# anibali/dsnt-pose2d

Hardware: AMD Instinct MI355X
Metric: images/sec (train step, 256x256, 16 joints) (higher is better)
Workload: dtype f32; 1 GPU; hg2 + DSNT + JS reg, 256x256 -> 64x64x16, batch 32 per GPU, RMSprop lr 2.5e-4, train step fwd+loss+bwd+optim; global_batch=32, parallelism=dp1, launches_fwd=212

## Files before the change

### dsnt-pose2d_amd/csrc/api.cpp

```cpp
#include "common.h"
#include "stage.h"
#include <string.h>

static thread_local char g_err[512] = "";

int dsnt_set_error(int code, const char* fmt, ...) {
    va_list ap;
    va_start(ap, fmt);
    vsnprintf(g_err, sizeof(g_err), fmt, ap);
    va_end(ap);
    return code;
}

int dsnt_device_id(void) {
    int d = 0;
    if (hipGetDevice(&d) != hipSuccess || d < 0) d = 0;
    return d < DSNT_MAX_DEVICES ? d : DSNT_MAX_DEVICES - 1;
}

int dsnt_device_cus(void) {
    static std::atomic<int> cus[DSNT_MAX_DEVICES];
    const int d = dsnt_device_id();
    int c = cus[d].load(std::memory_order_acquire);
    if (!c) {
        hipDeviceProp_t prop;
        int dev = 0;
        c = (hipGetDevice(&dev) == hipSuccess && hipGetDeviceProperties(&prop, dev) == hipSuccess && prop.multiProcessorCount > 0)
                ? prop.multiProcessorCount : 256;
        cus[d].store(c, std::memory_order_release);
    }
    return c;
}

extern "C" int dsnt_version(void) { return 124; }
extern "C" const char* dsnt_last_error(void) { return g_err; }

#include <vector>
#include <new>

struct dsnt_list {
    struct Entry {
        int kind;
        int lane, src, dst;
        mutable hipEvent_t ev;
        std::function<void(hipStream_t)> fn;
        int st_code = 0, gx = 0, gy = 0, nt = 0;
        std::vector<unsigned char> params;
        int fused = 0;
        unsigned* st_sync = nullptr;
    };
    std::vector<Entry> entries;
    std::vector<size_t> seg_start;
    dsnt_list() { seg_start.push_back(0); }
};

static thread_local dsnt_list* g_rec = nullptr;

dsnt_list* dsnt_recording(void) { return g_rec; }

void dsnt_record_launch(dsnt_list* l, int lane, std::function<void(hipStream_t)>&& fn) {
    dsnt_list::Entry e;
    e.kind = 0; e.lane = lane; e.src = e.dst = 0; e.ev = nullptr; e.fn = std::move(fn);
    l->entries.push_back(std::move(e));
}

void dsnt_record_launch_op(dsnt_list* l, int lane, std::function<void(hipStream_t)>&& fn, int code, int gx, int gy, int nt,
                           const void* params, size_t bytes) {
    dsnt_list::Entry e;
    e.kind = 0; e.lane = lane; e.src = e.dst = 0; e.ev = nullptr; e.fn = std::move(fn);
    if (code > 0 && code < DSNT_ST_CODES && bytes <= DSNT_STAGE_PARAM_BYTES && gx > 0 && gy > 0 && (nt == 256 || nt == DSNT_STAGE_NT || nt == 1024)) {
        e.st_code = code; e.gx = gx; e.gy = gy; e.nt = nt;
        e.params.assign((const unsigned char*)params, (const unsigned char*)params + bytes);
    }
    l->entries.push_back(std::move(e));
}

struct StageRun { std::vector<size_t> idx; int lane; int max_vb; };

static void stage_runs(const dsnt_list* l, int min_run, int max_vgrid, std::vector<StageRun>& runs) {
    std::vector<StageRun> open(DSNT_MAX_LANES);
    for (int i = 0; i < DSNT_MAX_LANES; ++i) { open[i].lane = i; open[i].max_vb = 0; }
    auto close = [&](int lane) {
        if ((int)open[lane].idx.size() >= min_run) runs.push_back(open[lane]);
        open[lane].idx.clear(); open[lane].max_vb = 0;
    };
    size_t next_seg = 1;
    for (size_t i = 0; i < l->entries.size(); ++i) {
// ... 164 lines not shown
```

### dsnt-pose2d_amd/csrc/conv_epilogue.h

```cpp
#pragma once
#include "conv_split.h"

template <int WM, int WN, int TM, int TN, bool HALO = false, int NT = 512>
__device__ __forceinline__ void conv_epilogue(const ConvP& p, f32x16 (&acc)[TM][TN], float* smem, int mtile,
                                              int ntile, int tid, int wave, int lane, int mbase = 0) {
    constexpr int BM = WM * TM * 32, BN = WN * TN * 32;
    auto rowmap = [&](int row) {
        return HALO ? mbase + (row >> 4) * p.W + (((row & 15) + ((row >> 4) & 1) * 14) & 15) : mtile * BM + row;
    };
    const int lr = lane & 31, lh = lane >> 5;
    const int cw = wave & 3;
    const int wm = cw / WN, wn = cw % WN;
    constexpr int CP = BN + 4;
    float* Cs = smem;
    if (wave < 4) {
#pragma unroll
        for (int a = 0; a < TM; ++a)
#pragma unroll
            for (int b = 0; b < TN; ++b) {
                const int col = (wn * TN + b) * 32 + lr;
                const int row0 = (wm * TM + a) * 32 + 4 * lh;
#pragma unroll
                for (int e = 0; e < 16; ++e)
                    Cs[(row0 + (e & 3) + 8 * (e >> 2)) * CP + col] = acc[a][b][e];
// ... 2 lines not shown
    __syncthreads();
    constexpr int CH = BN / 4;
    constexpr int RPP = NT / CH;
    constexpr int NPT = BM / RPP;
    constexpr int NP = NPT > 8 ? 8 : NPT;
    constexpr int NG = NPT / NP;
    const int ch = tid % CH, r0 = tid / CH;
    const int n0 = ntile * BN + ch * 4;
    const bool vn = n0 < p.Cout;
    float4 bias4 = make_float4(0.f, 0.f, 0.f, 0.f);
    if (p.bias && vn) bias4 = *reinterpret_cast<const float4*>(p.bias + n0);
    const bool bnb = p.bnb_scale != nullptr;
    float4 bsc = bias4, bsh = bias4, bmu = bias4, bis = bias4;
    if (bnb && vn) {
        bsc = *reinterpret_cast<const float4*>(p.bnb_scale + n0);
        bsh = *reinterpret_cast<const float4*>(p.bnb_shift + n0);
        bmu = *reinterpret_cast<const float4*>(p.bnb_mean + n0);
        bis = *reinterpret_cast<const float4*>(p.bnb_invstd + n0);
    } else if (p.tail.amax_bn && vn) {
        bsc = *reinterpret_cast<const float4*>(p.tail.amax_scale + n0);
        bsh = *reinterpret_cast<const float4*>(p.tail.amax_shift + n0);
    }
    const float am2lo = p.tail.amax_relu ? 0.f : -__builtin_inff();
    float am2 = 0.f;
    const float osc = p.a_bound ? 1.f / (pow2_scale(bound64(p.a_bound)) * pow2_scale(bound64(p.w_bound))) : 1.f;
    float4 s1 = make_float4(0.f, 0.f, 0.f, 0.f), s2 = s1;
    float am = 0.f;
#pragma unroll
    for (int gi = 0; gi < NG; ++gi) {
    float4 r1[NP], r2[NP];
#pragma unroll
    for (int j = 0; j < NP; ++j) {
        const int m = rowmap(r0 + RPP * (gi * NP + j));
        const bool ok = vn && m < p.M;
        const size_t o = ok ? (size_t)m * p.Cout + n0 : 0;
        r1[j] = p.res1 ? *reinterpret_cast<const float4*>(p.res1 + o) : make_float4(0.f, 0.f, 0.f, 0.f);
        r2[j] = p.res2 ? *reinterpret_cast<const float4*>(p.res2 + o) : make_float4(0.f, 0.f, 0.f, 0.f);
    }
#pragma unroll
    for (int j = 0; j < NP; ++j) {
        const int row = r0 + RPP * (gi * NP + j);
        const int m = rowmap(row);
        if (vn && m < p.M) {
            float4 v = *reinterpret_cast<const float4*>(Cs + row * CP + ch * 4);
            v.x *= osc; v.y *= osc; v.z *= osc; v.w *= osc;
            if (bnb) {
                const float4 xv = r1[j];
                if (p.bnb_relu) {
                    if (fmaf(xv.x, bsc.x, bsh.x) <= 0.f) v.x = 0.f;
                    if (fmaf(xv.y, bsc.y, bsh.y) <= 0.f) v.y = 0.f;
                    if (fmaf(xv.z, bsc.z, bsh.z) <= 0.f) v.z = 0.f;
                    if (fmaf(xv.w, bsc.w, bsh.w) <= 0.f) v.w = 0.f;
                }
                *reinterpret_cast<float4*>(p.y + (size_t)m * p.Cout + n0) = v;
                s1.x += v.x; s1.y += v.y; s1.z += v.z; s1.w += v.w;
                s2.x = fmaf(v.x, (xv.x - bmu.x) * bis.x, s2.x); s2.y = fmaf(v.y, (xv.y - bmu.y) * bis.y, s2.y);
                s2.z = fmaf(v.z, (xv.z - bmu.z) * bis.z, s2.z); s2.w = fmaf(v.w, (xv.w - bmu.w) * bis.w, s2.w);
                am = fmaxf(fmaxf(am, fabsf(v.x)), fmaxf(fabsf(v.y), fmaxf(fabsf(v.z), fabsf(v.w))));
                continue;
            }
            v.x += bias4.x + r1[j].x + r2[j].x; v.y += bias4.y + r1[j].y + r2[j].y;
            v.z += bias4.z + r1[j].z + r2[j].z; v.w += bias4.w + r1[j].w + r2[j].w;
            *reinterpret_cast<float4*>(p.y + (size_t)m * p.Cout + n0) = v;
            am = fmaxf(fmaxf(am, fabsf(v.x)), fmaxf(fabsf(v.y), fmaxf(fabsf(v.z), fabsf(v.w))));
            if (p.tail.amax_bn)
                am2 = fmaxf(fmaxf(am2, fabsf(fmaxf(fmaf(v.x, bsc.x, bsh.x), am2lo))),
                            fmaxf(fabsf(fmaxf(fmaf(v.y, bsc.y, bsh.y), am2lo)),
                                  fmaxf(fabsf(fmaxf(fmaf(v.z, bsc.z, bsh.z), am2lo)), fabsf(fmaxf(fmaf(v.w, bsc.w, bsh.w), am2lo)))));
            s1.x += v.x; s1.y += v.y; s1.z += v.z; s1.w += v.w;
            s2.x = fmaf(v.x, v.x, s2.x); s2.y = fmaf(v.y, v.y, s2.y);
            s2.z = fmaf(v.z, v.z, s2.z); s2.w = fmaf(v.w, v.w, s2.w);
        }
    }
    }
    if (p.tail.amax) amax_commit(am, p.tail.amax);
    if (p.tail.amax_bn) amax_commit(am2, p.tail.amax_bn, 1);
    if (p.stats) {
        __syncthreads();
        float* red = smem;
        float* mine = red + ((size_t)r0 * BN + ch * 4) * 2;
        mine[0] = s1.x; mine[1] = s2.x; mine[2] = s1.y; mine[3] = s2.y;
        mine[4] = s1.z; mine[5] = s2.z; mine[6] = s1.w; mine[7] = s2.w;
        __syncthreads();
        if (tid < BN) {
            const int n = ntile * BN + tid;
            if (n < p.Cout) {
                float a0 = 0.f, a1 = 0.f;
#pragma unroll
                for (int w = 0; w < RPP; ++w) {
                    a0 += red[((size_t)w * BN + tid) * 2 + 0];
                    a1 += red[((size_t)w * BN + tid) * 2 + 1];
                }
                tail_store(p.stats + ((size_t)mtile * 2 + 0) * p.Cout + n, a0);
                tail_store(p.stats + ((size_t)mtile * 2 + 1) * p.Cout + n, a1);
            }
        }
    }
}
```

### dsnt-pose2d_amd/csrc/conv_f32.hip

```cpp
#include "conv_epilogue.h"
#include "ew_bodies.h"
#include "stage.h"
#include <string.h>
#include <stdlib.h>

#define BK 32
#define PITCH 36

template <int WM, int WN, int TM, int TN, bool PRO, bool FAST>
__global__ __launch_bounds__(512, 4) void conv_fwd_kernel(ConvP p) {
    constexpr int BM = WM * TM * 32, BN = WN * TN * 32;
    constexpr int APASS = BM / 32, BPASS = BN / 32;
    extern __shared__ __attribute__((aligned(16))) float smem[];
    float* As = smem;
    float* Bs = smem + 2 * BM * PITCH;

    int tile;
    xcd_remap(blockIdx.x, p.mtiles * p.ntiles, tile);
    const int ntile = tile % p.ntiles, mtile = tile / p.ntiles;

    const int tid = threadIdx.x, lane = tid & 63;
    const int wave = __builtin_amdgcn_readfirstlane(tid >> 6);
    const int nsteps = (p.K + BK - 1) / BK;
    const int lr = lane & 31, lh = lane >> 5;
// ... 443 lines not shown
                p.y[o] = v;
                s1 += v;
                s2 = fmaf(v, (xv - bmu) * bis, s2);
            } else {
                v += bias + (PRO ? (p.res1 ? p.res1[o] : 0.f) : r1v[j]) + (p.res2 ? p.res2[o] : 0.f);
                p.y[o] = v;
                s1 += v;
                s2 = fmaf(v, v, s2);
            }
        }
    }
    if (p.stats) {
        __syncthreads();
        float* red = &part[0][0][0];
        red[(rg * 32 + col) * 2 + 0] = s1;
        red[(rg * 32 + col) * 2 + 1] = s2;
        __syncthreads();
        if (tid < 32 && vn) {
            float a0 = 0.f, a1 = 0.f;
#pragma unroll
            for (int w = 0; w < 16; ++w) { a0 += red[(w * 32 + tid) * 2 + 0]; a1 += red[(w * 32 + tid) * 2 + 1]; }
            tail_store(p.stats + ((size_t)mtile * 2 + 0) * p.Cout + n, a0);
            tail_store(p.stats + ((size_t)mtile * 2 + 1) * p.Cout + n, a1);
        }
    }
}
template <bool PRO, int CW>
__global__ __launch_bounds__(512) void conv_ksplit_kernel(ConvP p) {
    __shared__ __attribute__((aligned(16))) float part[8][32][33];
    conv_ksplit_body<PRO, CW>(p, blockIdx.x, part, true);
}

static long ksplit_rows() {
    static long v = -1;
    if (v < 0) {
        const char* e = getenv("DSNT_X_KSPLIT_ROWS");
        v = e ? atol(e) : 2048;
    }
    return v;
}

static bool conv_fwd_pro_ok(const dsnt_conv_geom* g, int tiles, int C) {
    return g && C == g->Cin && C <= 256 && C % 4 == 0 && tiles > 0 && (long)tiles * C <= 16384;
}
extern "C" int dsnt_conv_fwd_pro_ok(const dsnt_conv_geom* g, int tiles, int C) { return conv_fwd_pro_ok(g, tiles, C) ? 1 : 0; }

int conv_fill(ConvP& p, const char* who, const float* x, const void* w, bool planes, int64_t plane_stride, const float* bias,
              float* y, const float* in_scale, const float* in_shift, int in_relu, const float* res1, const float* res2,
              float* stats_partial, const dsnt_conv_geom* g, const dsnt_bn_bwd_epilogue* bnb, const dsnt_out_bounds* tail) {
    if (int e = conv_check_geom(g, who)) return e;
    char who_ex[64];
    snprintf(who_ex, sizeof(who_ex), "%s_ex", who);
    DSNT_REQUIRE(!bnb || (bnb->x && bnb->scale && bnb->shift && bnb->mean && bnb->invstd &&
                          stats_partial && !res1 && !res2 && !bias), DSNT_ERR_ARG,
                 "%s: the batch-norm-backward epilogue needs x/scale/shift/mean/invstd and "
                 "stats_partial, and excludes bias/residuals", who_ex);
    DSNT_REQUIRE(x && w && y, DSNT_ERR_ARG, "%s: null tensor", who);
    DSNT_REQUIRE((in_scale == nullptr) == (in_shift == nullptr), DSNT_ERR_ARG,
                 "%s: in_scale/in_shift must be given together", who);
    DSNT_REQUIRE(!planes || dsnt_conv_bf16x6_ok(g), DSNT_ERR_SHAPE,
                 "%s: geometry not supported (need Cin %% 16 == 0, <= 16 taps, < 2 GiB)", who);
    DSNT_REQUIRE(dsnt_aligned16(x) && dsnt_aligned16(w) && (!in_scale || dsnt_aligned16(in_scale)) &&
                 (!in_shift || dsnt_aligned16(in_shift)), DSNT_ERR_ALIGN,
                 "%s: x/w/scale/shift must be 16-byte aligned", who);
    DSNT_REQUIRE(!planes || (plane_stride >= (int64_t)g->Cout * g->R * g->S * g->Cin && plane_stride % 8 == 0 &&
                             (2 * plane_stride + (int64_t)g->Cout * g->R * g->S * g->Cin) * 2 < (1LL << 31)), DSNT_ERR_SHAPE,
                 "%s: bad plane stride %lld", who, (long long)plane_stride);
    p.x = x; p.bias = bias; p.y = y; p.in_scale = in_scale; p.in_shift = in_shift;
    p.w = planes ? nullptr : (const float*)w;
    p.wq = planes ? (const unsigned short*)w : nullptr; p.wq_stride = planes ? plane_stride : 0;
    p.res1 = res1; p.res2 = res2; p.stats = stats_partial; p.in_relu = in_relu;
    p.bnb_scale = p.bnb_shift = p.bnb_mean = p.bnb_invstd = nullptr; p.bnb_relu = 0;
    p.a_bound = p.w_bound = nullptr;
    p.ap_y = p.ap_scale = p.ap_mean = p.ap_invstd = p.ap_coef = nullptr; p.ap_out = nullptr;
    if (bnb) {
        p.res1 = bnb->x; p.bnb_scale = bnb->scale; p.bnb_shift = bnb->shift;
        p.bnb_mean = bnb->mean; p.bnb_invstd = bnb->invstd; p.bnb_relu = bnb->relu;
    }
    if (int e = out_bounds_fill(p.tail, tail, who_ex)) return e;
    DSNT_REQUIRE(!(p.tail.amax_bn && bnb), DSNT_ERR_ARG, "%s: dsnt_out_bounds.amax_bn excludes the batch-norm-backward epilogue", who_ex);
    memset(&p.pro, 0, sizeof(p.pro));
    conv_geom_fill(p, g);
    return DSNT_OK;
}

static int conv_fwd_impl(const float* x, const float* w, const float* bias, float* y,
                         const float* in_scale, const float* in_shift, int in_relu,
                         const float* res1, const float* res2, float* stats_partial,
                         const dsnt_conv_geom* g, const dsnt_bn_bwd_epilogue* g_bnb, const dsnt_out_bounds* g_tail,
                         void* stream, const dsnt_bn_prologue* g_pro = nullptr) {
    ConvP p;
    if (int e = conv_fill(p, "dsnt_conv_fwd", x, w, false, 0, bias, y, in_scale, in_shift, in_relu, res1, res2, stats_partial, g,
                          g_bnb, g_tail)) return e;
    if (g_pro) {
        DSNT_REQUIRE(g_pro->partial && g_pro->mean && g_pro->invstd && g_pro->scale && g_pro->shift && g_pro->M > 0 &&
                     conv_fwd_pro_ok(g, g_pro->tiles, g_pro->C), DSNT_ERR_ARG,
                     "dsnt_conv_fwd_pro: incomplete dsnt_bn_prologue, or more than 256 channels / 128 KB of partial sums");
        DSNT_REQUIRE((g_pro->running_mean == nullptr) == (g_pro->running_var == nullptr), DSNT_ERR_ARG,
                     "dsnt_conv_fwd_pro: running_mean/var must be given together");
        DSNT_REQUIRE(dsnt_aligned16(g_pro->scale) && dsnt_aligned16(g_pro->shift), DSNT_ERR_ALIGN, "dsnt_conv_fwd_pro: alignment");
        p.pro.partial = g_pro->partial; p.pro.tiles = g_pro->tiles; p.pro.C = g_pro->C;
        p.pro.invM = 1.0 / (double)g_pro->M;
        p.pro.unbias = g_pro->M > 1 ? (double)g_pro->M / (double)(g_pro->M - 1) : 1.0;
        p.pro.gamma = g_pro->gamma; p.pro.beta = g_pro->beta; p.pro.rmean = g_pro->running_mean; p.pro.rvar = g_pro->running_var;
        p.pro.momentum = g_pro->momentum; p.pro.eps = g_pro->eps;
        p.pro.mean = g_pro->mean; p.pro.invstd = g_pro->invstd; p.pro.scale = g_pro->scale; p.pro.shift = g_pro->shift;
    }
    int BM, BN;
    pick_cfg(g, BM, BN);
// ... 124 lines not shown
```

### dsnt-pose2d_amd/dsnt/engine.py

```python
import ctypes as C
import os
import struct

import torch

from . import _lib
from ._lib import ConvGeom, BnBwdEpilogue, BnTail, BnPrologue, BnBwdApply

BN_EPS = 1e-5
BN_MOMENTUM = 0.1


class Act:
    __slots__ = ('buf', 'N', 'H', 'W', 'C', '_grad', 'stats', 'name', 'grad_amax', 'amax_tail', 'fold_ok',
                 'pending_apply', 'uses', 'gives_away', 'is_branch', 'grad_shared', 'pending_add', 'base', 'base_amax')

    def __init__(self, buf, name=''):
        self.buf = buf
        self.N, self.H, self.W, self.C = buf.shape
        self._grad = None
        self.base, self.base_amax = None, None
        self.stats = None
        self.amax_tail = None
        self.grad_amax = None
        self.fold_ok = False
        self.pending_apply = None
        self.uses = 0
        self.gives_away = False
        self.is_branch = False
        self.grad_shared = False
        self.pending_add = None
        self.name = name

    @property
    def M(self):
        return self.N * self.H * self.W

    @property
    def grad(self):
        if self._grad is None and self.base is not None:
            self._grad, self.grad_amax, self.grad_shared = self.base, self.base_amax, True
        return self._grad

    @grad.setter
    def grad(self, g):
        self._grad = g


class ConvParams:
    __slots__ = ('w', 'b', 'gw', 'gb', 'Cout', 'R', 'S', 'Cin', 'stride', 'pad', 'dil', 'wq', 'wq_stride', 'wq16', 'wb',
                 'post_reduce')

    def __init__(self, w, b, gw, gb, stride=1, pad=0, dil=1):
        self.w, self.b, self.gw, self.gb = w, b, gw, gb
        self.wq, self.wq_stride = None, 0
        self.wq16, self.wb = None, None
        self.post_reduce = None
        self.Cout, self.R, self.S, self.Cin = w.shape
        self.stride, self.pad, self.dil = stride, pad, dil


class BnParams:
    __slots__ = ('gamma', 'beta', 'ggamma', 'gbeta', 'rmean', 'rvar', 'C', 'uses', 'momentum', 'eps')

    def __init__(self, gamma, beta, ggamma, gbeta, rmean, rvar, momentum=BN_MOMENTUM, eps=BN_EPS):
        self.gamma, self.beta, self.ggamma, self.gbeta = gamma, beta, ggamma, gbeta
        self.rmean, self.rvar = rmean, rvar
        self.momentum, self.eps = float(momentum), float(eps)
        self.C = gamma.numel()
        self.uses = 0


class Normed:
    __slots__ = ('x', 'bn', 'mean', 'invstd', 'scale', 'shift', 'relu', 'abound', 'pending', 'lane')


class _Conv:
    __slots__ = ('src', 'x', 'y', 'p', 'g', 'res1', 'res2', 'name', 'normed', 'sc', 'sh', 'relu', 'x_amax', 'use6', 'use16',
                 'slot', 'slot_k', 'bucket', 'fuse1', 'fold3_ok', 'need_input_grad', 'gd')


class _Dgrad:
    __slots__ = ('native', 'gd', 'gsrc', 'wd', 'wq', 'wq_stride', 'wq16', 'wbd', 'g_amax', 'd6', 'd16', 'd_stream')


class Tape:
    def __init__(self, device, training, record=None):
        self.device = device
        self.training = training
        self.record = training if record is None else bool(record)
        self.fwd = []
        self.bwd = []
        self._bwd_emitters = []
        self._scratch = {}
        self._keep = []
        self.lib = _lib.load()
        self.nbytes = 0
        self.bytes_fwd, self.bytes_bwd, self.bytes_by_name, self._ws_ptrs = 0, 0, {}, set()
        self._read_switches()
        self.lane = 0
        self.side_stream, self.wgrad_stream, self.more_streams = None, None, ()
        self.stage_census = []
        self._f16_w_stream = {}
        self.cur_bucket = 0
        self._wgrad_lane_reads = set()
        self._writer_base = None
        self._ident = None
        self._release_total, self._release_left, self._held = 0, 0, []
        self.acts = []
        self.dgrad_slots = []
        self.dgrad_total, self.dgrad_f32, self.dgrad_planes = 0, None, None
        self.param_arena = None
        self._pending_reduce = []
        self._pending_group = []
        self._f16_w_rows, self._f16_w_seen = [], set()
        self._f16_bn_rows = []
        self._eval_bn_rows = []
        self._amax_buf, self._amax_used = None, 0
        self._planar_src, self._prep_exempt, self._post_reduce = {}, set(), []
        self._famax_buf, self._famax_used, self._famax_of, self._famax_bn_of = None, 0, {}, {}
        self._f16_dw_rows = []
        self._dgrad_pack = None
        self.dgrad_planes16, self.dgrad_bounds = None, None
        self.f16_uses = []
        self._pending_group_uses = []
        self._clists = {}

    def _read_switches(self):
        self.use_bf16x6 = os.environ.get('DSNT_MFMA', 'bf16x6') != 'f32'
        self.bf16x6_min_rows = int(os.environ.get('DSNT_BF16X6_MIN_ROWS', '4096'))
        self.use_lanes = os.environ.get('DSNT_LANES', '1') != '0'
        self.side_lanes = (1, 3)
        self.n_lanes = 3 + len(self.side_lanes) - 1
        self.chain_lanes = (0,) + self.side_lanes
        self.wgrad_lane = 2 if (self.use_lanes and os.environ.get('DSNT_WGRAD_LANE', '1') != '0') else None
        self.wgrad_lane_rows = int(os.environ.get('DSNT_X_WGRAD_LANE_ROWS', '16000'))
        self.release_rows = int(os.environ.get('DSNT_X_RELEASE_ROWS', '4096'))
        off = set(os.environ.get('DSNT_OFF', '').replace('+', ',').split(','))
        self.conv3s = 'conv3s' not in off
        self.bwd1 = 'bwd1' not in off
        self.fwd1 = 'fwd1' not in off
        self.fold3 = 'fold3' not in off
        self.fold3_rows = int(os.environ.get('DSNT_X_FOLD3_ROWS', '16384'))
        self.stem4 = 'stem4' not in off
        self.stage = os.environ.get('DSNT_STAGE', '0') == '1'
        self.stage_min_run = int(os.environ.get('DSNT_X_STAGE_MIN_RUN', '3'))
        self.stage_max_vgrid = int(os.environ.get('DSNT_X_STAGE_MAX_VGRID', '512'))
        self.stage_grid = int(os.environ.get('DSNT_X_STAGE_GRID', '64'))
        self._x = dict(kv.split('=') for kv in os.environ.get('DSNT_X', '').split(',') if '=' in kv)
        self.wgrad_narrow = self._x.get('wgrad_narrow', '1')
        self.share_grads = self._x.get('share_grads', '1') != '0'
        self.defer_res = self._x.get('defer_res', '1') != '0'
        self.flush_points = self._x.get('flush_points', '1') != '0'
        self.prep_split = self._x.get('prep_split', '1') != '0'
        self.defer_reduce = os.environ.get('DSNT_DEFER_REDUCE', '1') != '0'
        self.group_rows = int(os.environ.get('DSNT_X_GROUP_ROWS', '8192')) if self.defer_reduce else 0
        self.fuse_finalize = os.environ.get('DSNT_FUSE_FINALIZE', '1') != '0'
        self.fuse_finalize_max = int(os.environ.get('DSNT_X_FUSE_FINALIZE_MAX', '2048'))
        self.use_f16x3 = self.use_bf16x6 and os.environ.get('DSNT_SPLIT', 'f16x3') == 'f16x3'
        if self.record and not self.training:
            self.use_f16x3 = False

    def empty(self, *shape, dtype=torch.float32):
        t = torch.empty(*shape, device=self.device, dtype=dtype)
        self.nbytes += t.numel() * t.element_size()
        self._keep.append(t)
        return t

    def scratch(self, key, numel, dtype=torch.float32, least=1):
        key = (key, self.lane)
        t = self._scratch.get(key)
        if t is None or t.numel() < numel:
            if t is not None:
                self._keep.append(t)
            t = torch.empty(max(numel, least), device=self.device, dtype=dtype)
            self.nbytes += t.numel() * t.element_size()
            self._scratch[key] = t
        return t

    def f16_weights(self, p, wq16=None, wsrc=None, wb=None, stream=False):
        wq16 = p.wq16 if wq16 is None else wq16
        key = wq16.data_ptr()
        if key not in self._f16_w_seen:
            self._f16_w_seen.add(key)
            wsrc = p.w if wsrc is None else wsrc
            wb = p.wb if wb is None else wb
            n = wsrc.numel()
            assert n % 4 == 0
            self._f16_w_rows.append([wsrc.data_ptr(), wq16.data_ptr(), wb.data_ptr(), n, p.wq_stride] +
                                    ([p.Cout, p.Cin] if stream else [0, 0]))
            self._f16_w_stream[key] = stream
        assert self._f16_w_stream.get(key, False) == stream, 'one weight tensor, two plane layouts'

    def stream_ok(self, p, g, rows, res2):
        return (self.conv3s and p.R == 3 and p.S == 3 and res2 is None and
                bool(self.lib.dsnt_conv_fwd_stream_ok(C.byref(g))))
# ... 409 lines not shown
        acc = 1
        if a.grad is None:
            a.grad = self.empty(a.N, a.H, a.W, a.C)
            acc = 0
        elif a.grad.data_ptr() in self._wgrad_lane_reads:
            self._wgrad_lane_reads.discard(a.grad.data_ptr())
            self.release_wgrads()
            self.sync_bwd(self.wgrad_lane, self.lane)
        if self.use_f16x3 and amax:
            if a.grad_amax is None:
                a.grad_amax = self.amax_slot()
        else:
            a.grad_amax = None
        return a.grad, acc

    def grad_identity(self, a, g, donate, g_amax=None):
        if a.pending_apply is not None:
            self.materialize_apply(a)
        if a.pending_add is not None:
            self._flush_add(a)
        if a.grad is None and donate:
            a.grad = g
            a.grad_amax = g_amax
            return True
        buf, acc = self.grad_target(a, amax=True)
        if a.grad_amax is not None:
            self.b('dsnt_axpy_amax', g, buf, 1.0, acc, g.numel(), a.grad_amax)
        else:
            self.b('dsnt_axpy', g, buf, 1.0, acc, g.numel())
        return False

    def geom(self, x, p):
        Ho = (x.H + 2 * p.pad - p.dil * (p.R - 1) - 1) // p.stride + 1
        Wo = (x.W + 2 * p.pad - p.dil * (p.S - 1) - 1) // p.stride + 1
        assert x.C == p.Cin, (x.C, p.Cin)
        return ConvGeom(x.N, x.H, x.W, p.Cin, Ho, Wo, p.Cout, p.R, p.S, p.stride, p.pad, p.dil)

    def ensure_stats(self, a):
        if a.stats is None:
            tiles = (a.M + 127) // 128
            part = self.empty(tiles, 2, a.C)
            self.f('dsnt_bn_stats', a.buf, part, a.M, a.C)
            a.stats = (part, tiles)
        return a.stats

    def norm(self, x, bn, relu=True):
        if os.environ.get('DSNT_DEBUG_NO_RELU'):
            relu = False
        n = Normed()
        n.x, n.bn, n.relu = x, bn, relu
        n.abound = None
        n.mean, n.invstd, n.scale, n.shift = (self.empty(bn.C) for _ in range(4))
        n.pending = None
        n.lane = self.lane
        if self.training:
            part, tiles = self.ensure_stats(x)
            if self.fuse_finalize and bn.C <= 256 and tiles * bn.C <= self.fuse_finalize_max:
                n.pending = (part, tiles)
            else:
                self.f('dsnt_bn_finalize', part, tiles, x.M, bn.C, bn.gamma, bn.beta, bn.rmean, bn.rvar,
                       bn.momentum, bn.eps, 1, n.mean, n.invstd, n.scale, n.shift)
        else:
            bits = struct.unpack('<I', struct.pack('<f', float(bn.eps)))[0]
            self._eval_bn_rows.append([bn.gamma.data_ptr(), bn.beta.data_ptr(), bn.rmean.data_ptr(), bn.rvar.data_ptr(),
                                       n.mean.data_ptr(), n.invstd.data_ptr(), n.scale.data_ptr(), n.shift.data_ptr(),
                                       bn.C, bits])
        return n

    def check_lane(self, n):
        if n.pending is not None:
            n.lane = self.lane
        elif n.lane != self.lane:
            raise RuntimeError('dsnt: BatchNorm vectors finalised on lane %d are read on lane %d without a synchronisation '
                               '(trace norm() and its consumers on one lane, or sync the lanes)' % (n.lane, self.lane))

    def materialize(self, n):
        self.check_lane(n)
        if n.pending is not None:
            part, tiles = n.pending
            n.pending = None
            bn = n.bn
            self.f('dsnt_bn_finalize', part, tiles, n.x.M, bn.C, bn.gamma, bn.beta, bn.rmean, bn.rvar,
                   bn.momentum, bn.eps, 1, n.mean, n.invstd, n.scale, n.shift)

    def fold_ok(self, n):
        x = n.x
        return bool(self.bwd1 and x.fold_ok and x.grad is None and x.pending_apply is None)

    def materialize_apply(self, x):
        ap, x.pending_apply = x.pending_apply, None
        n = ap['n']
        buf, acc = self.grad_target(x, amax=True)
        if x.grad_amax is not None:
            self.b('dsnt_bn_act_bwd_apply_amax', ap['dz'], x.buf, n.scale, n.shift, n.mean, n.invstd, ap['coef'], 0,
                   buf, acc, x.M, n.bn.C, x.grad_amax)
        else:
            self.b('dsnt_bn_act_bwd_apply', ap['dz'], x.buf, n.scale, n.shift, n.mean, n.invstd, ap['coef'], 0,
                   buf, acc, x.M, n.bn.C)

    def _norm_backward(self, n, da, reduced=None, finalised=False, dz_amax=None):
        x, bn = n.x, n.bn
        coef = self.scratch('bncoef', 2 * bn.C)
        relu = 1 if n.relu else 0
        if reduced is not None:
            part, tiles = reduced
            relu = 0
        else:
            tiles = (x.M + 127) // 128
            part = self.scratch('bnpart', tiles * 2 * bn.C).view(-1)
            self.b('dsnt_bn_act_bwd_reduce', da, x.buf, n.scale, n.shift, n.mean, n.invstd, relu, part,
                   x.M, bn.C)
        if dz_amax is not None:
            assert reduced is not None and not finalised and x.grad is None
            acc_p = 1 if bn.uses > 0 else 0
            bn.uses += 1
            coef = self.empty(2 * bn.C)
            bound = self.amax_slot()
            self.b('dsnt_bn_bwd_finalize_bound', part, tiles, x.M, bn.C, bn.ggamma, bn.gbeta, acc_p, coef, n.scale,
                   dz_amax, bound)
            x.pending_apply = dict(dz=da, n=n, coef=coef, bound=bound, dz_amax=dz_amax)
            return
        frozen = not self.training
        fused = (not finalised) and self.fuse_finalize and bn.C <= 256 and tiles * bn.C <= self.fuse_finalize_max and not frozen
        assert not (frozen and finalised)
        if not finalised:
            acc_p = 1 if bn.uses > 0 else 0
            bn.uses += 1
            if not fused:
                self.b('dsnt_bn_bwd_finalize', part, tiles, x.M, bn.C, bn.ggamma, bn.gbeta, acc_p | (2 if frozen else 0), coef)
        buf, acc = self.grad_target(x, amax=True, base_ok=True)
        base = self.take_base()
        if fused:
            coef = self.empty(2 * bn.C)
            if base is not None:
                self.b('dsnt_bn_act_bwd_apply_pro_base', da, x.buf, n.scale, n.shift, n.mean, n.invstd, part, tiles,
                       bn.ggamma, bn.gbeta, acc_p, coef, relu, base, buf, x.M, bn.C, x.grad_amax)
            else:
                self.b('dsnt_bn_act_bwd_apply_pro', da, x.buf, n.scale, n.shift, n.mean, n.invstd, part, tiles,
                       bn.ggamma, bn.gbeta, acc_p, coef, relu, buf, acc, x.M, bn.C, x.grad_amax)
        elif base is not None:
            self.b('dsnt_bn_act_bwd_apply_base', da, x.buf, n.scale, n.shift, n.mean, n.invstd, coef, relu,
                   base, buf, x.M, bn.C, x.grad_amax)
        elif x.grad_amax is not None:
            self.b('dsnt_bn_act_bwd_apply_amax', da, x.buf, n.scale, n.shift, n.mean, n.invstd, coef, relu,
                   buf, acc, x.M, bn.C, x.grad_amax)
        else:
            self.b('dsnt_bn_act_bwd_apply', da, x.buf, n.scale, n.shift, n.mean, n.invstd, coef, relu,
                   buf, acc, x.M, bn.C)

    def conv(self, src, p, res1=None, res2=None, want_stats=False, need_input_grad=True, name=''):
        c = _Conv()
        c.src, c.p, c.res1, c.res2, c.name, c.need_input_grad = src, p, res1, res2, name, need_input_grad
        c.normed = isinstance(src, Normed)
        c.x = x = src.x if c.normed else src
        c.g = self.geom(x, p)
        c.y = y = self.act(x.N, c.g.Ho, c.g.Wo, p.Cout, name)
        x.uses += 1
        for r in (res1, res2):
            if r is not None:
                r.uses += 1
                y.gives_away = True
        c.sc, c.sh, c.relu = (src.scale, src.shift, 1 if src.relu else 0) if c.normed else (None, None, 0)
        self._conv_forward(c, want_stats)
        if self.record:
            self._conv_backward_plan(c)
            self.on_backward(lambda: self._conv_backward(c))
        return y

    def _share(self, persistent=True):
        return 2 if (persistent and self.lane != 0) else 0

    def _operand_bound(self, c):
        return self.operand_amax_bn(c.src) if c.normed else self.operand_amax(c.x)

    @staticmethod
    def _bn_epilogue(x, n):
        vectors = (n.scale, n.shift, n.mean, n.invstd) if n is not None else (None,) * 4
        return BnBwdEpilogue(_lib.ptr(x.buf), *(_lib.ptr(v) for v in vectors), 1 if (n is not None and n.relu) else 0)

    @staticmethod
    def _bn_apply(y, ap):
        n = ap['n']
        return (BnBwdApply(_lib.ptr(y.buf), _lib.ptr(n.scale), _lib.ptr(n.mean), _lib.ptr(n.invstd), _lib.ptr(ap['coef'])),
                dict(dz=ap['dz'], y=y.buf, scale=n.scale, mean=n.mean, invstd=n.invstd, coef=ap['coef']))

    def _dz_buffer(self, x, private):
        n = x.M * x.C
        return self.empty(n) if private else self.scratch('da', n).view(-1)[:n]

    def _reduce_row(self, ws, p, splits):
        self._pending_reduce.append([ws.data_ptr(), p.gw.data_ptr(), p.gb.data_ptr() if p.gb is not None else 0,
                                     splits, p.Cout * p.R * p.S * p.Cin, p.Cout, 0])

    def _struct_bytes(self, name, nb):
        self.bytes_bwd += nb
        self.bytes_by_name[name] = self.bytes_by_name.get(name, 0) + nb

    def _conv_forward(self, c, want_stats):
        src, x, y, p, g, normed, res2 = c.src, c.x, c.y, c.p, c.g, c.normed, c.res2
        sc, sh, relu = c.sc, c.sh, c.relu
        if normed:
            self.check_lane(src)
        part, tail = None, None
        use6 = c.use6 = self._use6(g) and p.wq is not None
        can16 = use6 and p.wq16 is not None
        early = can16 and p.R == 1 and res2 is None and self.fwd1
        x_amax = self._operand_bound(c) if early else None
# ... 26 lines not shown
            ab = self.f16_bn_bound(src) if (normed and self.training) else x_amax
            if f1:
                e = self.f('dsnt_conv1x1_fwd_f16x3', x.buf, p.wq16, p.wq_stride, p.wb, ab, p.b, y.buf, sc, sh, relu | f1_shr, r1,
                           part, g, tail)
            elif s4:
                e = self.f('dsnt_stem4_fwd_f16x3', x.buf, p.wq16, p.wq_stride, p.wb, ab, p.b, y.buf, part, g, tail)
            else:
                e = self.f('dsnt_conv_fwd_f16x3_stream' if st else 'dsnt_conv_fwd_f16x3_ex', x.buf, p.wq16, p.wq_stride, p.wb, ab,
                           p.b, y.buf, sc, sh, relu | self._share(st or p.R == 1), r1, r2, part, g, None, tail)
            self.f16_uses.append((e, dict(kind='fwd', name=c.name, x=x.buf, sc=sc, sh=sh, relu=relu, a_bound=ab,
                                          w=p.w, w_bound=p.wb)))
        elif use6:
            self.f('dsnt_conv_fwd_bf16x6_ex', x.buf, p.wq, p.wq_stride, p.b, y.buf, sc, sh, relu, r1, r2, part, g,
                   None, tail)
        elif normed and src.pending is not None and self.lib.dsnt_conv_fwd_pro_ok(C.byref(g), src.pending[1], src.bn.C):
            spart, stiles = src.pending
            src.pending = None
            bn = src.bn
            pro = BnPrologue(_lib.ptr(spart), stiles, bn.C, x.M, _lib.ptr(bn.gamma), _lib.ptr(bn.beta), _lib.ptr(bn.rmean),
                             _lib.ptr(bn.rvar), bn.momentum, bn.eps, _lib.ptr(src.mean), _lib.ptr(src.invstd),
                             _lib.ptr(src.scale), _lib.ptr(src.shift))
            self._keep.extend((spart, src.mean, src.invstd, src.scale, src.shift))
            self.f('dsnt_conv_fwd_pro', x.buf, p.w, p.b, y.buf, pro, relu, r1, r2, part, g, tail)
        else:
            if normed:
                self.materialize(src)
            self.f('dsnt_conv_fwd_ex', x.buf, p.w, p.b, y.buf, sc, sh, relu, r1, r2, part, g, None, tail)

    def _conv_backward_plan(self, c):
        x, y, p, g = c.x, c.y, c.p, c.g
        c.slot = c.slot_k = None
        if c.need_input_grad and self.param_arena is not None:
            c.slot, c.slot_k = self.dgrad_total, len(self.dgrad_slots)
            self.dgrad_slots.append((p, c.slot))
            self.dgrad_total += (p.w.numel() + 7) // 8 * 8
        c.bucket = self.cur_bucket
        one_pass = self.bwd1 and self.use_f16x3 and self.defer_reduce and c.slot is not None
        c.fuse1 = bool(one_pass and (c.normed or c.x_amax is not None) and p.R == 1 and p.S == 1 and p.post_reduce is None and
                       self.lib.dsnt_conv1x1_bwd_ok(C.byref(g)))
        plain = c.normed and c.res1 is None and c.res2 is None
        c.gd = None
        if p.stride == 1:
            c.gd = ConvGeom(x.N, g.Ho, g.Wo, p.Cout, x.H, x.W, p.Cin, p.R, p.S, 1, p.dil * (p.R - 1) - p.pad, p.dil)
        c.fold3_ok = bool(self.fold3 and one_pass and plain and self.training and p.R == 3 and p.S == 3 and c.gd is not None and
                          c.use16 and y.M >= self.fold3_rows and self._use6(c.gd) and self.stream_ok(p, c.gd, x.M, None))
        y.fold_ok = bool(c.fuse1 and plain) or c.fold3_ok

    def _conv_backward(self, c):
        y = c.y
        gy, ap = y.grad, y.pending_apply
        fused = c.fuse1 and self.dgrad_planes16 is not None
        fold3 = bool(c.fold3_ok and ap is not None and gy is None and self.dgrad_planes16 is not None and c.need_input_grad and
                     ap['bound'] is not None)
        if ap is not None and (not fused or gy is not None) and not fold3:
            self.materialize_apply(y)
            ap, gy = None, y.grad
        assert gy is not None or ap is not None, 'no gradient reached conv output ' + c.name
        if fused and ap is None and y.grad_amax is None:
            fused = False
        wl, defer_res = self.lane, False
        if fused:
            self._conv_bwd_fused1(c, ap, gy)
        elif fold3:
            gy = y._grad = self.empty(y.N, y.H, y.W, y.C)
            y.grad_amax, y.pending_apply = ap['bound'], None
            self._conv_dgrad(c, gy, ap)
            wl, defer_res = self._conv_wgrad(c, gy)
        else:
            wl, defer_res = self._conv_wgrad(c, gy)
            self._conv_dgrad(c, gy, None)
        self._conv_residual_grads(c, gy, wl, defer_res)

    def _conv_bwd_fused1(self, c, ap, gy):
        src, x, y, p, g, name = c.src, c.x, c.y, c.p, c.g, 'dsnt_conv1x1_bwd_f16x3'
        nw = p.w.numel()
        shr = self._share()
        nsp = self.lib.dsnt_conv1x1_bwd_splits(C.byref(g), shr)
        ws = self.empty(self.lib.dsnt_conv1x1_bwd_ws_floats(C.byref(g), shr))
        self._ws_ptrs.add(ws.data_ptr())
        wd = self.dgrad_f32[c.slot:c.slot + nw]
        wq16 = self.dgrad_planes16[c.slot:c.slot + nw]
        wbd = self.dgrad_bounds[64 * c.slot_k:64 * c.slot_k + 64]
        self._f16_dw_rows.append([wd.data_ptr(), wq16.data_ptr(), wbd.data_ptr(), nw, self.dgrad_total, 0, 0])
        if ap is not None:
            aps, applied = self._bn_apply(y, ap)
            dy, gb = ap['dz'], ap['bound']
            y.pending_apply = None
            grad = dict(g_apply=applied, g_bound=gb)
        else:
            aps, dy, gb = None, gy, y.grad_amax
            grad = dict(g=dy, g_bound=gb)
        if c.normed:
            ab = self.f16_bn_bound_bwd(src)
            fold = self.fold_ok(src)
            dz = self._dz_buffer(x, fold)
            dz_amax = self.amax_slot() if fold else None
            part = self.scratch('bnpart', nsp * 2 * x.C).view(-1)
            e = self.b(name, self._bn_epilogue(x, src), dy, aps, wq16, self.dgrad_total, wbd, ab, gb, dz, part, ws, dz_amax, shr, g)
        else:
            ab = c.x_amax
            buf, acc = self.grad_target(x, amax=True)
            e = self.b(name, self._bn_epilogue(x, None), dy, None, wq16, self.dgrad_total, wbd, ab, gb, buf, None, ws,
                       x.grad_amax, shr | acc, g)
        self._struct_bytes(name, 4 * (x.buf.numel() + (y.buf.numel() if ap is not None else 0)))
        u = dict(kind='bwd1', name=c.name, x=x.buf, sc=c.sc, sh=c.sh, relu=c.relu, a_bound=ab, w=wd, w_bound=wbd)
        u.update(grad)
        self.f16_uses.append((e, u))
        self._reduce_row(ws, p, nsp)
        if c.normed:
            self._norm_backward(src, dz, reduced=(part, nsp), finalised=False, dz_amax=dz_amax)

    def _conv_wgrad(self, c, gy):
        p, g = c.p, c.g
        cur = wl = self.lane
        if self.wgrad_lane is not None and (self.wgrad_lane_rows == 0 or (
                cur in self.chain_lanes and c.res1 is None and c.res2 is None and g.N * g.Ho * g.Wo >= self.wgrad_lane_rows)):
            wl = self.wgrad_lane
        hold = wl != cur and self._release_left > 0
        if hold:
            listed, self.bwd = self.bwd, self._held
        self.sync_bwd(cur, wl)
        self.lane = wl
        if wl != cur:
            self._wgrad_lane_reads.add(gy.data_ptr())
        share = 2 if (wl != cur and c.need_input_grad) else 0
        if share and self.wgrad_narrow in ('1', {0: '2'}.get(c.bucket, '3')):
            share |= 4
        w6 = self.use_bf16x6 and bool(self.lib.dsnt_conv_wgrad_bf16x6_ok(C.byref(g)))
        defer_res = False
        if self.defer_reduce:
            defer_res = self._conv_wgrad_slab(c, gy, share, w6, wl == cur)
        else:
            ws = self.scratch('wgrad', self.lib.dsnt_conv_wgrad_ws_floats(C.byref(g)))
            self.b('dsnt_conv_wgrad_bf16x6' if w6 else 'dsnt_conv_wgrad', c.x.buf, c.sc, c.sh, c.relu, gy, ws, p.gw, p.gb, 0, g)
            if p.post_reduce is not None:
                self.b(p.post_reduce[0], *p.post_reduce[1])
        self.lane = cur
        if hold:
            self.bwd = listed
        return wl, defer_res

    def _conv_wgrad_slab(self, c, gy, share, w6, on_chain):
        x, y, p, g, normed, sc, sh, relu = c.x, c.y, c.p, c.g, c.normed, c.sc, c.sh, c.relu
        groupable = (w6 and (normed or self.share_grads) and on_chain and not y.grad_shared and
                     0 < g.N * g.Ho * g.Wo <= self.group_rows)
        residuals = [r for r in (c.res1, c.res2) if r is not None]
        defer_res = bool(groupable and residuals and self.share_grads and self.defer_res and all(
            r._grad is None and r.base is None and r.pending_apply is None and r.pending_add is None for r in residuals))
        grouped = groupable and (not residuals or defer_res)
        w16 = w6 and self.use_f16x3 and (normed or c.x_amax is not None) and y.grad_amax is not None
        ab = (self.f16_bn_bound_bwd(c.src) if normed else c.x_amax) if w16 else None
        if w16 and not grouped:
            nws = self.lib.dsnt_conv_wgrad_f16x3_ws_floats(C.byref(g), share)
            splits = self.lib.dsnt_conv_wgrad_f16x3_splits(C.byref(g), share)
        else:
            nws, splits = self.lib.dsnt_conv_wgrad_ws_floats(C.byref(g)), self.lib.dsnt_conv_wgrad_splits(C.byref(g))
        ws = self.empty(nws)
        self._ws_ptrs.add(ws.data_ptr())
        use = dict(kind='wgrad', name=c.name, x=x.buf, sc=sc, sh=sh, relu=relu, a_bound=ab, g=gy, g_bound=y.grad_amax)
        if grouped:
            desc = C.create_string_buffer(self.lib.dsnt_conv_wgrad_desc_bytes())
            gsc, gsh = (sc, sh) if normed else self.identity_bn(x.C)
            if w16:
# ... 2 lines not shown
                self._pending_group_uses.append(use)
            else:
                nblk = self.lib.dsnt_conv_wgrad_desc(_lib.ptr(x.buf), _lib.ptr(gsc), _lib.ptr(gsh), relu, _lib.ptr(gy),
                                                     _lib.ptr(ws), C.byref(g), desc)
            if nblk <= 0:
                raise RuntimeError('dsnt_conv_wgrad_desc failed: %s' % self.lib.dsnt_last_error().decode())
            self._pending_group.append((desc.raw, nblk))
        elif w16:
            e = self.b('dsnt_conv_wgrad_f16x3', x.buf, sc, sh, relu, gy, ws, None, None, share, ab, y.grad_amax, g)
            self.f16_uses.append((e, use))
        else:
            self.b('dsnt_conv_wgrad_bf16x6' if w6 else 'dsnt_conv_wgrad', x.buf, sc, sh, relu, gy, ws, None, None,
                   share if w6 else 0, g)
        if p.post_reduce is not None:
            self._post_reduce.append(p.post_reduce)
        self._reduce_row(ws, p, splits)
        return defer_res

    def _conv_dgrad_operands(self, c, gy):
        x, p, g = c.x, c.p, c.g
        d = _Dgrad()
        nw = p.w.numel()
        pad_d = p.dil * (p.R - 1) - p.pad
        assert pad_d >= 0, 'data gradient needs pad <= dil * (R - 1)'
        d.native = p.stride != 1 and c.slot is not None and self.lib.dsnt_conv_dgrad_strided_ok(C.byref(g))
        d.gd, d.gsrc = c.gd, gy
        if p.stride != 1 and not d.native:
            Hs, Ws = x.H + 2 * p.pad - p.dil * (p.R - 1), x.W + 2 * p.pad - p.dil * (p.S - 1)
            d.gsrc = self.scratch('stuffed', x.N * Hs * Ws * p.Cout).view(-1)[:x.N * Hs * Ws * p.Cout]
            self.b('dsnt_zero_insert', gy, d.gsrc, x.N, g.Ho, g.Wo, p.Cout, Hs, Ws, p.stride)
            d.gd = ConvGeom(x.N, Hs, Ws, p.Cout, x.H, x.W, p.Cin, p.R, p.S, 1, pad_d, p.dil)
        d.wq = d.wq_stride = d.wq16 = d.wbd = d.d_stream = None
        if c.slot is not None:
            d.wd = self.dgrad_f32[c.slot:c.slot + nw]
            d.wq, d.wq_stride = self.dgrad_planes[c.slot:c.slot + nw], self.dgrad_total
            d.d6 = d.gd is not None and self._use6(d.gd)
        else:
            d.wd = self.scratch('wdgrad', nw)
            self.b('dsnt_conv_pack_dgrad', p.w, d.wd, p.Cout, p.R, p.S, p.Cin)
            d.d6 = self._use6(d.gd) and nw % 8 == 0
            if d.d6:
                d.wq, d.wq_stride = self.scratch('wdgrad6', 3 * nw, torch.bfloat16, 8), nw
                self.b('dsnt_split_bf16x3', d.wd, d.wq, nw)
        d.g_amax = c.y.grad_amax if (self.use_f16x3 and p.stride == 1) else None
        d.d16 = d.d6 and d.g_amax is not None and c.slot is not None and self.dgrad_planes16 is not None
        if d.d16:
            d.wq16 = self.dgrad_planes16[c.slot:c.slot + nw]
            d.wbd = self.dgrad_bounds[64 * c.slot_k:64 * c.slot_k + 64]
            d.d_stream = self.stream_ok(p, d.gd, x.M, None)
            self._f16_dw_rows.append([d.wd.data_ptr(), d.wq16.data_ptr(), d.wbd.data_ptr(), nw, self.dgrad_total] +
                                     ([p.Cin, p.Cout] if d.d_stream else [0, 0]))
        return d

    def _conv_dgrad_launch(self, c, d, out, res, part=None, bnb=None, tail=None):
        if d.native:
            self.b('dsnt_conv_dgrad_strided', d.gsrc, d.wd, out, res, part, c.g, bnb, tail)
        elif d.d16:
            e = self.b('dsnt_conv_fwd_f16x3_stream' if d.d_stream else 'dsnt_conv_fwd_f16x3_ex', d.gsrc, d.wq16, self.dgrad_total,
                       d.wbd, d.g_amax, None, out, None, None, self._share(d.d_stream or c.p.R == 1), res, None, part, d.gd, bnb, tail)
            self.f16_uses.append((e, dict(kind='dgrad', name=c.name, g=d.gsrc, g_bound=d.g_amax, w=d.wd, w_bound=d.wbd)))
        elif d.d6:
            self.b('dsnt_conv_fwd_bf16x6_ex', d.gsrc, d.wq, d.wq_stride, None, out, None, None, 0, res, None, part, d.gd, bnb, tail)
        else:
            self.b('dsnt_conv_fwd_ex', d.gsrc, d.wd, None, out, None, None, 0, res, None, part, d.gd, bnb, tail)

    def _conv_dgrad(self, c, gy, ap):
        if not c.need_input_grad:
            return
        src, x, y = c.src, c.x, c.y
        d = self._conv_dgrad_operands(c, gy)
        if not c.normed:
            buf, acc = self.grad_target(x, amax=bool(d.d6 or d.native), base_ok=True)
            base = self.take_base()
            tl = None
            if x.grad_amax is not None:
                tl = BnTail()
                tl.amax = x.grad_amax.data_ptr()
            self._conv_dgrad_launch(c, d, buf, base if base is not None else (buf if acc else None), tail=tl)
            return
        fold = not d.native and self.fold_ok(src)
        dz = self._dz_buffer(x, fold)
        if d.native:
            tiles = self.lib.dsnt_conv_dgrad_strided_tiles(C.byref(c.g))
        else:
            bm = 128 if d.d6 else self.lib.dsnt_conv_fwd_bm(C.byref(d.gd))
            tiles = (x.M + bm - 1) // bm
        part = self.scratch('bnpart', tiles * 2 * x.C).view(-1)
        bnb = self._bn_epilogue(x, src)
        tl, dz_amax = None, None
        if fold:
            tl, dz_amax = BnTail(), self.amax_slot()
            tl.amax = dz_amax.data_ptr()
        if ap is not None:
            assert d.d16 and d.d_stream and not d.native
            name = 'dsnt_conv_dgrad_f16x3_stream_apply'
            aps, applied = self._bn_apply(y, ap)
            e = self.b(name, ap['dz'], aps, gy, d.wq16, self.dgrad_total, d.wbd, ap['bound'], dz, part, self._share(), d.gd, bnb, tl)
            self._struct_bytes(name, 4 * y.buf.numel())
            self.f16_uses.append((e, dict(kind='dgrad', name=c.name, w=d.wd, w_bound=d.wbd, g_bound=ap['bound'], g_apply=applied)))
        else:
            self._conv_dgrad_launch(c, d, dz, None, part, bnb, tl)
        self._norm_backward(src, dz, reduced=(part, tiles), dz_amax=dz_amax)

    def _conv_residual_grads(self, c, gy, wl, defer_res):
        y = c.y
        if c.res1 is not None or c.res2 is not None:
            self.sync_bwd(wl, self.lane)
        donated = False
        for r in (c.res1, c.res2):
            if r is None:
                continue
            if defer_res:
                r.base, r.base_amax = gy, y.grad_amax
            elif (donated and self.share_grads and r.grad is None and r.pending_apply is None and r.uses == 1 and
                    not r.gives_away and not r.is_branch):
                r.grad, r.grad_amax, r.grad_shared = gy, y.grad_amax, True
            else:
                donated = self.grad_identity(r, gy, donate=not donated, g_amax=y.grad_amax) or donated

    def _f_with_stats(self, name, y, tensors, dims):
        part = None
        if self.training:
            tiles = (y.M + 127) // 128
            part = self.empty(tiles, 2, y.C)
            y.stats = (part, tiles)
        if self.use_f16x3 and y.M >= self.bf16x6_min_rows:
            y.amax_tail = BnTail()
        if part is None and y.amax_tail is None:
            self.f(name, *tensors, *dims)
        else:
            self.f(name + '_stats', *tensors, part, *dims, y.amax_tail)

    def bn_act(self, x, bn, relu=True, name=''):
        n = self.norm(x, bn, relu)
        self.materialize(n)
        y = self.act(x.N, x.H, x.W, x.C, name)
        x.uses += 1
        self._f_with_stats('dsnt_bn_act_fwd', y, (x.buf, n.scale, n.shift, 1 if n.relu else 0, y.buf), (x.M, x.C))
        if self.record:
            def backward():
                self._norm_backward(n, y.grad)
            self.on_backward(backward)
        return y

    def maxpool2(self, x, name=''):
        y = self.act(x.N, x.H // 2, x.W // 2, x.C, name)
        x.uses += 1
        idx = self.empty(x.N, x.H // 2, x.W // 2, x.C, dtype=torch.uint8)
        self._f_with_stats('dsnt_maxpool2_fwd', y, (x.buf, y.buf, idx), (x.N, x.H, x.W, x.C))
        if self.record:
            def backward():
                add, x.pending_add = x.pending_add, None
                buf, acc = self.grad_target(x, amax=True, take_add=True)
                if add is not None:
                    assert acc == 1
# ... 117 lines not shown
```

Before: 2937 images/sec.

## Fold second BN-backward consumer's dz into dgrad epilogue via res2 accumulation

When a batch-norm output feeds two convolutions, the first conv's dgrad now leaves its raw dz and partial statistics pending instead of applying BN backward right away. The second conv's bf16x6 dgrad then adds that earlier dz through the res2 input of its BN-backward epilogue, so one apply pass covers both branches. The aim is to cut a separate BN-backward reduce/apply pass and a gradient accumulation over the activation. In exchange it adds tracking state, extra finalize launches on the fallback path, and a looser argument check that allows res2 together with the BN epilogue.

```diff
diff --git a/dsnt-pose2d_amd/csrc/api.cpp b/dsnt-pose2d_amd/csrc/api.cpp
--- a/dsnt-pose2d_amd/csrc/api.cpp
+++ b/dsnt-pose2d_amd/csrc/api.cpp
@@ -32,7 +32,7 @@
     return c;
 }
 
-extern "C" int dsnt_version(void) { return 124; }
+extern "C" int dsnt_version(void) { return 125; }
 extern "C" const char* dsnt_last_error(void) { return g_err; }
 
 #include <vector>
diff --git a/dsnt-pose2d_amd/csrc/conv_epilogue.h b/dsnt-pose2d_amd/csrc/conv_epilogue.h
--- a/dsnt-pose2d_amd/csrc/conv_epilogue.h
+++ b/dsnt-pose2d_amd/csrc/conv_epilogue.h
@@ -78,6 +78,7 @@
                     if (fmaf(xv.z, bsc.z, bsh.z) <= 0.f) v.z = 0.f;
                     if (fmaf(xv.w, bsc.w, bsh.w) <= 0.f) v.w = 0.f;
                 }
+                if (p.res2) { v.x += r2[j].x; v.y += r2[j].y; v.z += r2[j].z; v.w += r2[j].w; }
                 *reinterpret_cast<float4*>(p.y + (size_t)m * p.Cout + n0) = v;
                 s1.x += v.x; s1.y += v.y; s1.z += v.z; s1.w += v.w;
                 s2.x = fmaf(v.x, (xv.x - bmu.x) * bis.x, s2.x); s2.y = fmaf(v.y, (xv.y - bmu.y) * bis.y, s2.y);
diff --git a/dsnt-pose2d_amd/csrc/conv_f32.hip b/dsnt-pose2d_amd/csrc/conv_f32.hip
--- a/dsnt-pose2d_amd/csrc/conv_f32.hip
+++ b/dsnt-pose2d_amd/csrc/conv_f32.hip
@@ -519,9 +519,9 @@
     char who_ex[64];
     snprintf(who_ex, sizeof(who_ex), "%s_ex", who);
     DSNT_REQUIRE(!bnb || (bnb->x && bnb->scale && bnb->shift && bnb->mean && bnb->invstd &&
-                          stats_partial && !res1 && !res2 && !bias), DSNT_ERR_ARG,
+                          stats_partial && !res1 && (!res2 || planes) && !bias), DSNT_ERR_ARG,
                  "%s: the batch-norm-backward epilogue needs x/scale/shift/mean/invstd and "
-                 "stats_partial, and excludes bias/residuals", who_ex);
+                 "stats_partial, and excludes bias/residuals (res2 = an earlier dz: the split-precision tiled kernels only)", who_ex);
     DSNT_REQUIRE(x && w && y, DSNT_ERR_ARG, "%s: null tensor", who);
     DSNT_REQUIRE((in_scale == nullptr) == (in_shift == nullptr), DSNT_ERR_ARG,
                  "%s: in_scale/in_shift must be given together", who);
diff --git a/dsnt-pose2d_amd/dsnt/engine.py b/dsnt-pose2d_amd/dsnt/engine.py
--- a/dsnt-pose2d_amd/dsnt/engine.py
+++ b/dsnt-pose2d_amd/dsnt/engine.py
@@ -72,7 +72,7 @@
 
 
 class Normed:
-    __slots__ = ('x', 'bn', 'mean', 'invstd', 'scale', 'shift', 'relu', 'abound', 'pending', 'lane')
+    __slots__ = ('x', 'bn', 'mean', 'invstd', 'scale', 'shift', 'relu', 'abound', 'pending', 'lane', 'nuse', 'ndone')
 
 
 class _Conv:
@@ -142,6 +142,7 @@
         self.fwd1 = 'fwd1' not in off
         self.fold3 = 'fold3' not in off
         self.fold3_rows = int(os.environ.get('DSNT_X_FOLD3_ROWS', '16384'))
+        self.foldraw = 'foldraw' not in off
         self.stem4 = 'stem4' not in off
         self.stage = os.environ.get('DSNT_STAGE', '0') == '1'
         self.stage_min_run = int(os.environ.get('DSNT_X_STAGE_MIN_RUN', '3'))
@@ -657,6 +658,7 @@
         n.abound = None
         n.mean, n.invstd, n.scale, n.shift = (self.empty(bn.C) for _ in range(4))
         n.pending = None
+        n.nuse, n.ndone = 0, 0
         n.lane = self.lane
         if self.training:
             part, tiles = self.ensure_stats(x)
@@ -692,9 +694,26 @@
         x = n.x
         return bool(self.bwd1 and x.fold_ok and x.grad is None and x.pending_apply is None)
 
+    def fold_opens(self, n):
+        x = n.x
+        return bool(self.foldraw and self.training and n.nuse == 2 and n.ndone == 0 and self.use_bf16x6 and
+                    x.M >= self.bf16x6_min_rows and not self.fold_ok(n) and x._grad is None and x.base is None and
+                    x.pending_apply is None and x.pending_add is None)
+
+    def fold_joins(self, n, d):
+        ap = n.x.pending_apply
+        return bool(ap is not None and ap.get('open') and ap['n'] is n and ap['lane'] == self.lane and n.ndone == 1 and
+                    n.x.grad is None and d.d6 and not d.native and not d.d_stream)
+
     def materialize_apply(self, x):
         ap, x.pending_apply = x.pending_apply, None
         n = ap['n']
+        if ap.get('open'):
+            bn = n.bn
+            ap['coef'] = self.empty(2 * bn.C)
+            self.b('dsnt_bn_bwd_finalize', ap['part'], ap['tiles'], x.M, bn.C, bn.ggamma, bn.gbeta, 1 if bn.uses > 0 else 0,
+                   ap['coef'])
+            bn.uses += 1
         buf, acc = self.grad_target(x, amax=True)
         if x.grad_amax is not None:
             self.b('dsnt_bn_act_bwd_apply_amax', ap['dz'], x.buf, n.scale, n.shift, n.mean, n.invstd, ap['coef'], 0,
@@ -703,8 +722,9 @@
             self.b('dsnt_bn_act_bwd_apply', ap['dz'], x.buf, n.scale, n.shift, n.mean, n.invstd, ap['coef'], 0,
                    buf, acc, x.M, n.bn.C)
 
-    def _norm_backward(self, n, da, reduced=None, finalised=False, dz_amax=None):
+    def _norm_backward(self, n, da, reduced=None, finalised=False, dz_amax=None, opens=False):
         x, bn = n.x, n.bn
+        n.ndone += 1
         coef = self.scratch('bncoef', 2 * bn.C)
         relu = 1 if n.relu else 0
         if reduced is not None:
@@ -715,6 +735,11 @@
             part = self.scratch('bnpart', tiles * 2 * bn.C).view(-1)
             self.b('dsnt_bn_act_bwd_reduce', da, x.buf, n.scale, n.shift, n.mean, n.invstd, relu, part,
                    x.M, bn.C)
+        if opens:
+            assert reduced is not None and not finalised and dz_amax is None and x.grad is None
+            x.pending_apply = dict(dz=da, n=n, coef=None, bound=None, dz_amax=None, open=True, part=part, tiles=tiles,
+                                   lane=self.lane)
+            return
         if dz_amax is not None:
             assert reduced is not None and not finalised and x.grad is None
             acc_p = 1 if bn.uses > 0 else 0
@@ -758,6 +783,8 @@
         c.src, c.p, c.res1, c.res2, c.name, c.need_input_grad = src, p, res1, res2, name, need_input_grad
         c.normed = isinstance(src, Normed)
         c.x = x = src.x if c.normed else src
+        if c.normed:
+            src.nuse += 1
         c.g = self.geom(x, p)
         c.y = y = self.act(x.N, c.g.Ho, c.g.Wo, p.Cout, name)
         x.uses += 1
@@ -890,7 +917,7 @@
         fused = c.fuse1 and self.dgrad_planes16 is not None
         fold3 = bool(c.fold3_ok and ap is not None and gy is None and self.dgrad_planes16 is not None and c.need_input_grad and
                      ap['bound'] is not None)
-        if ap is not None and (not fused or gy is not None) and not fold3:
+        if ap is not None and (not fused or gy is not None or ap.get('open')) and not fold3:
             self.materialize_apply(y)
             ap, gy = None, y.grad
         assert gy is not None or ap is not None, 'no gradient reached conv output ' + c.name
@@ -931,9 +958,10 @@
         if c.normed:
             ab = self.f16_bn_bound_bwd(src)
             fold = self.fold_ok(src)
-            dz = self._dz_buffer(x, fold)
+            opens = self.fold_opens(src)
+            dz = self._dz_buffer(x, fold or opens)
             dz_amax = self.amax_slot() if fold else None
-            part = self.scratch('bnpart', nsp * 2 * x.C).view(-1)
+            part = self.empty(nsp * 2 * x.C) if opens else self.scratch('bnpart', nsp * 2 * x.C).view(-1)
             e = self.b(name, self._bn_epilogue(x, src), dy, aps, wq16, self.dgrad_total, wbd, ab, gb, dz, part, ws, dz_amax, shr, g)
         else:
             ab = c.x_amax
@@ -946,7 +974,7 @@
         self.f16_uses.append((e, u))
         self._reduce_row(ws, p, nsp)
         if c.normed:
-            self._norm_backward(src, dz, reduced=(part, nsp), finalised=False, dz_amax=dz_amax)
+            self._norm_backward(src, dz, reduced=(part, nsp), finalised=False, dz_amax=dz_amax, opens=opens)
 
     def _conv_wgrad(self, c, gy):
         p, g = c.p, c.g
@@ -1055,15 +1083,16 @@
                                      ([p.Cin, p.Cout] if d.d_stream else [0, 0]))
         return d
 
-    def _conv_dgrad_launch(self, c, d, out, res, part=None, bnb=None, tail=None):
+    def _conv_dgrad_launch(self, c, d, out, res, part=None, bnb=None, tail=None, res2=None):
+        assert res2 is None or (d.d6 and not d.native and not d.d_stream)
         if d.native:
             self.b('dsnt_conv_dgrad_strided', d.gsrc, d.wd, out, res, part, c.g, bnb, tail)
         elif d.d16:
             e = self.b('dsnt_conv_fwd_f16x3_stream' if d.d_stream else 'dsnt_conv_fwd_f16x3_ex', d.gsrc, d.wq16, self.dgrad_total,
-                       d.wbd, d.g_amax, None, out, None, None, self._share(d.d_stream or c.p.R == 1), res, None, part, d.gd, bnb, tail)
+                       d.wbd, d.g_amax, None, out, None, None, self._share(d.d_stream or c.p.R == 1), res, res2, part, d.gd, bnb, tail)
             self.f16_uses.append((e, dict(kind='dgrad', name=c.name, g=d.gsrc, g_bound=d.g_amax, w=d.wd, w_bound=d.wbd)))
         elif d.d6:
-            self.b('dsnt_conv_fwd_bf16x6_ex', d.gsrc, d.wq, d.wq_stride, None, out, None, None, 0, res, None, part, d.gd, bnb, tail)
+            self.b('dsnt_conv_fwd_bf16x6_ex', d.gsrc, d.wq, d.wq_stride, None, out, None, None, 0, res, res2, part, d.gd, bnb, tail)
         else:
             self.b('dsnt_conv_fwd_ex', d.gsrc, d.wd, None, out, None, None, 0, res, None, part, d.gd, bnb, tail)
 
@@ -1081,14 +1110,19 @@
                 tl.amax = x.grad_amax.data_ptr()
             self._conv_dgrad_launch(c, d, buf, base if base is not None else (buf if acc else None), tail=tl)
             return
+        join = ap is None and self.fold_joins(src, d)
+        dz1 = None
+        if join:
+            dz1, x.pending_apply = x.pending_apply['dz'], None
         fold = not d.native and self.fold_ok(src)
-        dz = self._dz_buffer(x, fold)
+        opens = not d.native and self.fold_opens(src)
+        dz = self._dz_buffer(x, fold or opens)
         if d.native:
             tiles = self.lib.dsnt_conv_dgrad_strided_tiles(C.byref(c.g))
         else:
             bm = 128 if d.d6 else self.lib.dsnt_conv_fwd_bm(C.byref(d.gd))
             tiles = (x.M + bm - 1) // bm
-        part = self.scratch('bnpart', tiles * 2 * x.C).view(-1)
+        part = self.empty(tiles * 2 * x.C) if opens else self.scratch('bnpart', tiles * 2 * x.C).view(-1)
         bnb = self._bn_epilogue(x, src)
         tl, dz_amax = None, None
         if fold:
@@ -1102,8 +1136,8 @@
             self._struct_bytes(name, 4 * y.buf.numel())
             self.f16_uses.append((e, dict(kind='dgrad', name=c.name, w=d.wd, w_bound=d.wbd, g_bound=ap['bound'], g_apply=applied)))
         else:
-            self._conv_dgrad_launch(c, d, dz, None, part, bnb, tl)
-        self._norm_backward(src, dz, reduced=(part, tiles), dz_amax=dz_amax)
+            self._conv_dgrad_launch(c, d, dz, None, part, bnb, tl, res2=dz1)
+        self._norm_backward(src, dz, reduced=(part, tiles), dz_amax=dz_amax, opens=opens)
 
     def _conv_residual_grads(self, c, gy, wl, defer_res):
         y = c.y
```

After: 2958 images/sec (median of 6 runs). Within noise of the previous version (+0.7%).
